# SinOncology/BreakID

Measured on AMD Instinct MI355X. Metric: M reads/s clustered+split-scanned, higher is better.
Workload: dtype int32/u8 (+f64 sd replay)

## Files before the change

### breakid_amd/capi.py

```python
from __future__ import annotations

import ctypes as C
import math
import os
import subprocess

import numpy as np

from . import abi

_HERE = os.path.dirname(os.path.abspath(__file__))
LIB_PATH = os.path.join(_HERE, "libbreakid_hip.so")
_LIB = None


class BreakIDError(RuntimeError):
    def __init__(self, code, msg):
        super().__init__("libbreakid_hip error %d: %s" % (code, msg))
        self.code = code


def build(verbose=False):
    cmd = ["make", "-C", os.path.join(_HERE, "csrc"), "-j8"]
    r = subprocess.run(cmd, capture_output=not verbose, text=True)
    if r.returncode != 0:
        raise RuntimeError("building libbreakid_hip.so failed:\n" + (r.stdout or "")[-4000:] + (r.stderr or "")[-4000:])


EXPORTS = ["bk_init", "bk_prepare_process", "bk_free", "bk_last_error", "bk_set_stream", "bk_sync", "bk_get_stream", "bk_upload_records", "bk_records", "bk_exclude_regions", "bk_isize_stats",
           "bk_discordant_pairs", "bk_mask_and_cluster", "bk_split_evidence", "bk_cluster_summary",
           "bk_split_breakpoints", "bk_normal_support", "bk_ref_support", "bk_genotype_call", "bk_clip_support", "bk_clip_reads", "bk_base_depth", "bk_clip_rescue", "bk_junctions", "bk_junction_sides", "bk_vcf_breakend_alt", "bk_evidence", "bk_run", "bk_fetch", "bk_timing", "bk_timing_enable", "bk_timing_touched", "bk_group_stats", "bk_qname_hash", "bk_qname_check",
           "bk_bam_open", "bk_bam_header", "bk_bam_decode", "bk_bam_close", "bk_bam_extract", "bk_bam_names_free", "bk_bam_decode_device", "bk_bam_decode_device_part", "bk_bam_decode_device_ctx", "bk_bam_dev_free", "bk_feed_release_caches", "bk_debug_bgzf_inflate", "bk_debug_std_sort", "bk_sort_forms", "bk_debug_ahc", "bk_debug_points", "bk_debug_cigar", "bk_debug_vote", "bk_debug_region", "bk_shard_begin", "bk_shard_get_stats", "bk_shard_set_stats",
           "bk_shard_sd_local", "bk_shard_sd_finish", "bk_shard_buffer", "bk_shard_set_buffer", "bk_shard_group_sizes",
           "bk_shard_own_groups", "bk_shard_route_candidates", "bk_shard_group_keys", "bk_shard_route_pairs", "bk_shard_group_pairs", "bk_shard_bp_cov", "bk_shard_bp_vote", "bk_shard_bp_vote_slice", "bk_shard_bp_set_voted", "bk_shard_bp_depth", "bk_shard_bp_finish"]


def lib():
    global _LIB
    if _LIB is None:
        if not os.path.exists(LIB_PATH):
            raise BreakIDError(abi.BK_ERR_NO_DEVICE, "libbreakid_hip.so is not built (run __graft_entry__.build()); "
                                                     "there is no CPU fallback")
        try:
            import torch
        except Exception:
            pass
        L = C.CDLL(LIB_PATH)
        vp, u64p, dp = C.c_void_p, C.POINTER(C.c_uint64), C.POINTER(C.c_double)
        L.bk_init.argtypes = [C.c_int, vp, C.POINTER(C.c_char_p), C.c_int, C.POINTER(vp)]
        L.bk_free.argtypes = [vp]
        L.bk_last_error.restype = C.c_char_p
        L.bk_last_error.argtypes = [vp]
        L.bk_set_stream.argtypes = [vp, vp]
        L.bk_sync.argtypes = [vp]
        L.bk_upload_records.argtypes = [vp, C.POINTER(abi.Soa), C.c_int]
        L.bk_records.argtypes = [vp, C.POINTER(abi.Soa)]
        L.bk_exclude_regions.argtypes = [vp, C.POINTER(abi.Regions), u64p]
        L.bk_isize_stats.argtypes = [vp, dp, dp]
        L.bk_discordant_pairs.argtypes = [vp, C.c_int, C.c_double, u64p, C.POINTER(C.c_uint32)]
        L.bk_mask_and_cluster.argtypes = [vp, C.c_double, C.c_int, u64p]
        L.bk_split_evidence.argtypes = [vp, u64p]
        L.bk_cluster_summary.argtypes = [vp, C.c_double, u64p]
        L.bk_split_breakpoints.argtypes = [vp, C.c_double, u64p]
        L.bk_run.argtypes = [vp, C.c_int, C.c_int, dp, u64p]
        L.bk_normal_support.argtypes = [vp, vp, C.c_double, C.POINTER(vp), u64p]
        L.bk_ref_support.argtypes = [vp, vp, C.c_int, C.c_int, C.c_double, C.POINTER(vp), u64p]
        L.bk_genotype_call.argtypes = [C.c_uint32, C.c_uint32, C.POINTER(C.c_uint8), C.POINTER(C.c_uint8), C.POINTER(C.c_float)]
        L.bk_clip_support.argtypes = [vp, vp, C.c_int, C.c_int, C.c_double, C.POINTER(vp), u64p]
        L.bk_clip_reads.argtypes = [vp, vp, C.c_uint64, C.c_int, C.c_int, C.POINTER(vp), C.POINTER(vp), C.POINTER(vp)]
        L.bk_base_depth.argtypes = [vp, vp, vp, C.c_uint64, C.POINTER(vp)]
        L.bk_clip_rescue.argtypes = [vp, vp, vp, C.c_uint32] + [C.POINTER(C.c_uint32)] * 4
        L.bk_junctions.argtypes = [vp, C.POINTER(vp), u64p]
        L.bk_junction_sides.argtypes = [vp, C.POINTER(C.c_uint8), C.POINTER(C.c_uint8), C.POINTER(C.c_uint8)]
        L.bk_vcf_breakend_alt.argtypes = [C.c_char, C.c_int, C.c_char_p, C.c_uint32, C.c_int, C.c_char_p, C.c_size_t]
        L.bk_evidence.argtypes = [vp, C.POINTER(vp), u64p, C.POINTER(C.POINTER(C.c_uint64))]
        L.bk_fetch.argtypes = [vp, C.c_int, C.POINTER(vp), u64p, C.POINTER(C.POINTER(C.c_uint64)), C.POINTER(C.c_uint32)]
        L.bk_timing.argtypes = [vp, C.POINTER(C.POINTER(C.c_char_p)), C.POINTER(C.POINTER(C.c_float)),
                                C.POINTER(C.POINTER(C.c_uint64)), C.POINTER(C.c_int)]
        L.bk_timing_enable.argtypes = [vp, C.c_int]
        L.bk_timing_touched.argtypes = [vp, C.POINTER(C.POINTER(C.c_uint64)), C.POINTER(C.c_int)]
        L.bk_debug_std_sort.argtypes = [vp, vp, vp, C.c_uint32, vp]
        L.bk_sort_forms.argtypes = [vp, u64p]
        L.bk_debug_ahc.argtypes = [vp, vp, vp, C.c_uint32, C.c_double, vp, vp, C.POINTER(C.c_uint32)]
        L.bk_debug_points.argtypes = [vp, C.c_int, vp, vp, C.c_uint32, C.c_double, vp, vp, C.POINTER(C.c_uint32)]
        L.bk_debug_cigar.argtypes = [vp, C.c_uint32, vp, vp, vp, vp, vp, vp, vp]
        L.bk_debug_vote.argtypes = [vp, vp, C.c_uint32, vp, C.c_uint32, C.c_int32, C.c_int32, vp]
        L.bk_debug_region.argtypes = [vp, C.c_int32, C.c_uint32, C.c_uint32, C.c_uint64, vp, C.c_uint32, C.POINTER(C.c_uint32), C.POINTER(C.c_uint32),
                                      C.POINTER(C.c_uint32)]
        L.bk_shard_begin.argtypes = [vp, C.c_uint64, C.c_int]
        L.bk_shard_get_stats.argtypes = [vp, C.POINTER(abi.ShardStats)]
        L.bk_shard_set_stats.argtypes = [vp, C.POINTER(abi.ShardStats)]
        L.bk_shard_sd_local.argtypes = [vp, u64p, C.POINTER(vp), u64p]
        L.bk_shard_sd_finish.argtypes = [vp, vp, C.c_uint64, C.c_uint64, dp, dp]
        L.bk_shard_buffer.argtypes = [vp, C.c_int, C.POINTER(vp), u64p, C.POINTER(C.c_uint32)]
        L.bk_shard_set_buffer.argtypes = [vp, C.c_int, vp, C.c_uint64]
        L.bk_shard_group_sizes.argtypes = [vp, C.POINTER(C.POINTER(C.c_uint64)), C.POINTER(C.c_uint32)]
        L.bk_shard_own_groups.argtypes = [vp, vp, C.c_uint32]
        L.bk_shard_route_candidates.argtypes = [vp, C.c_uint32, C.POINTER(vp), C.POINTER(C.POINTER(C.c_uint64))]
        L.bk_shard_group_keys.argtypes = [vp, C.POINTER(C.POINTER(C.c_uint32)), C.POINTER(C.c_uint32)]
        L.bk_shard_route_pairs.argtypes = [vp, vp, C.c_uint32, C.c_uint32, C.POINTER(vp), C.POINTER(C.POINTER(C.c_uint64))]
        L.bk_shard_group_pairs.argtypes = [vp, vp, C.c_uint64, vp, C.c_uint32]
        L.bk_shard_bp_cov.argtypes = [vp, C.c_double, C.POINTER(vp), u64p]
        L.bk_shard_bp_vote.argtypes = [vp, C.c_double, vp]
        L.bk_shard_bp_vote_slice.argtypes = [vp, C.c_double, vp, C.c_uint64, C.c_uint64, C.POINTER(vp), C.POINTER(vp)]
        L.bk_shard_bp_set_voted.argtypes = [vp, vp]
        L.bk_shard_bp_depth.argtypes = [vp, C.POINTER(vp), u64p]
        L.bk_shard_bp_finish.argtypes = [vp, vp]
        L.bk_qname_hash.restype = C.c_uint64
        L.bk_qname_hash.argtypes = [C.c_char_p, C.c_size_t]
        L.bk_qname_check.restype = C.c_uint32
        L.bk_qname_check.argtypes = [C.c_char_p, C.c_size_t]
        L.bk_bam_open.argtypes = [C.c_char_p, C.POINTER(vp), C.c_char_p, C.c_size_t]
        L.bk_bam_header.argtypes = [vp, C.POINTER(C.c_int), C.POINTER(C.POINTER(C.c_char_p)), C.POINTER(C.POINTER(C.c_uint32))]
        L.bk_bam_decode.argtypes = [vp, C.POINTER(abi.Soa), C.c_char_p, C.c_size_t]
        L.bk_bam_close.argtypes = [vp]
        L.bk_bam_extract.argtypes = [C.c_char_p, C.c_char_p, vp, C.c_uint64, C.POINTER(C.c_char_p), C.c_uint64, C.POINTER(vp), u64p, C.c_char_p, C.c_size_t]
        L.bk_bam_names_free.argtypes = [vp]
        L.bk_bam_names_free.restype = None
        L.bk_bam_decode_device.argtypes = [C.c_char_p, C.c_int, C.POINTER(vp), C.POINTER(abi.Soa), C.POINTER(C.c_int), C.POINTER(C.POINTER(C.c_char_p)),
                                           C.POINTER(C.POINTER(C.c_uint32)), C.c_char_p, C.c_size_t]
        L.bk_bam_decode_device_part.argtypes = [C.c_char_p, C.c_int, C.c_int, C.c_int, C.POINTER(vp), C.POINTER(abi.Soa), C.POINTER(C.c_int), C.POINTER(C.POINTER(C.c_char_p)),
                                           C.POINTER(C.POINTER(C.c_uint32)), C.c_char_p, C.c_size_t]
        L.bk_bam_dev_free.argtypes = [vp]
        L.bk_feed_release_caches.argtypes = []
        L.bk_feed_release_caches.restype = None
        L.bk_bam_decode_device_ctx.argtypes = [C.c_char_p, C.c_int, C.c_int, C.POINTER(vp), C.POINTER(vp), C.POINTER(C.c_int), C.POINTER(C.POINTER(C.c_char_p)),
                                               C.POINTER(C.POINTER(C.c_uint32)), C.c_char_p, C.c_size_t]
        L.bk_debug_bgzf_inflate.argtypes = [vp, C.c_uint64, vp, C.c_uint64, C.POINTER(C.c_uint64), C.POINTER(C.c_float), C.c_char_p, C.c_size_t]
        _LIB = L
    return _LIB


MULTI_LIB_PATH = os.path.join(_HERE, "libbreakid_rccl.so")
_MULTI = None
TRANSPORT_AUTO, TRANSPORT_RCCL, TRANSPORT_LOCAL = 0, 1, 2


def multi_lib():
    global _MULTI
    if _MULTI is None:
        lib()
        if not os.path.exists(MULTI_LIB_PATH):
            raise BreakIDError(abi.BK_ERR_NO_DEVICE, "libbreakid_rccl.so is not built (run __graft_entry__.build())")
        M = C.CDLL(MULTI_LIB_PATH)
        vp, dp = C.c_void_p, C.POINTER(C.c_double)
        M.bk_multi_run.argtypes = [C.POINTER(abi.Soa), vp, C.POINTER(C.c_char_p), C.c_int, C.c_int, C.c_int, C.c_int, C.c_int, dp, C.POINTER(C.c_uint64), C.POINTER(vp),
                                   C.c_char_p, C.c_size_t]
        M.bk_multi_stats.argtypes = [vp, dp, dp, C.POINTER(vp), C.POINTER(C.c_uint32)]
        M.bk_multi_free.argtypes = [vp]
        M.bk_multi_free.restype = None
        _MULTI = M
    return _MULTI


def multi_run(contigs, cols, n_gpus, transport=TRANSPORT_LOCAL, qual=20, fast=True):
    M = multi_lib()
    qc = cols.get("qcheck")
    cols = {k: np.ascontiguousarray(cols[k], dtype=dt) for k, dt in abi.SOA_COLS}
    if qc is not None:
        cols["qcheck"] = np.ascontiguousarray(qc, dtype=np.uint32)
    for k in ("cigar", "aux"):
        if cols[k].size == 0:
            cols[k] = np.zeros(1, cols[k].dtype)
    soa = abi.soa_from_numpy(cols)
    lens = np.asarray([l for _, l in contigs], dtype=np.uint32)
    names = (C.c_char_p * len(contigs))(*[n.encode() for n, _ in contigs])
    w, ncl, h = C.c_double(), C.c_uint64(), C.c_void_p()
    err = C.create_string_buffer(512)
    rc = M.bk_multi_run(C.byref(soa), lens.ctypes.data, names, len(contigs), int(n_gpus), int(transport), int(qual), int(fast), C.byref(w), C.byref(ncl), C.byref(h), err, 512)
    if rc != 0:
        raise BreakIDError(rc, err.value.decode())
    try:
        mean, sd = C.c_double(), C.c_double()
        rc = M.bk_multi_stats(h, C.byref(mean), C.byref(sd), None, None)
        if rc != 0:
            raise BreakIDError(rc, "bk_multi_stats")
        L = lib()
        clusters, _ = abi.fetch_array(L, h, lambda hh, st, d, c, g, ng: L.bk_fetch(hh, st, d, c, g, ng), abi.STAGE_CLUSTERS)
        return {"w": w.value, "n_clustered": ncl.value, "mean": mean.value, "sd": sd.value, "clusters": clusters}
    finally:
        M.bk_multi_free(h)


def w_from(mean, sd):
    times = 2
    return times * math.sqrt(times) * (mean + 3 * sd)


def genotype_call(alt, ref):
    gt, gq, vaf = C.c_uint8(), C.c_uint8(), C.c_float()
    rc = lib().bk_genotype_call(int(alt), int(ref), C.byref(gt), C.byref(gq), C.byref(vaf))
    if rc != 0:
        raise BreakIDError(rc, "bk_genotype_call")
    return gt.value, gq.value, np.float32(vaf.value)


def junction_sides(row):
    a = np.zeros(1, abi.JUNCTION)
    a[0] = row
    r1, r2, src = C.c_uint8(), C.c_uint8(), C.c_uint8()
    rc = lib().bk_junction_sides(a.ctypes.data, C.byref(r1), C.byref(r2), C.byref(src))
    if rc != 0:
        raise BreakIDError(rc, "bk_junction_sides")
    return r1.value, r2.value, src.value


def clip_rescue(cluster, junction, clip, min_support=3):
    c, j, s = np.zeros(1, abi.CLUSTER), np.zeros(1, abi.JUNCTION), np.zeros(1, abi.CLIP_SUPPORT)
    c[0], j[0], s[0] = cluster, junction, clip
    out = [C.c_uint32() for _ in range(4)]
    rc = lib().bk_clip_rescue(c.ctypes.data, j.ctypes.data, s.ctypes.data, int(min_support), *[C.byref(o) for o in out])
    if rc < 0:
        raise BreakIDError(rc, "bk_clip_rescue")
    return tuple(o.value for o in out) if rc == 1 else None


def vcf_breakend_alt(ref_base, own_right, mate_chr, mate_pos, mate_right, cap=None):
    chrom = mate_chr.encode()
    if cap is None:
        cap = len(chrom) + 32
    buf = C.create_string_buffer(max(int(cap), 1))
    rc = lib().bk_vcf_breakend_alt(ref_base.encode(), int(bool(own_right)), chrom, int(mate_pos), int(bool(mate_right)), buf, int(cap))
    if rc != 0:
        raise BreakIDError(rc, "bk_vcf_breakend_alt")
    return buf.value.decode()


class Context:

    def __init__(self, contigs, device=0):
        self.L = lib()
        self.contigs = list(contigs)
        lens = np.asarray([l for _, l in contigs], dtype=np.uint32)
        names = (C.c_char_p * len(contigs))(*[n.encode() for n, _ in contigs])
        h = C.c_void_p()
        rc = self.L.bk_init(device, lens.ctypes.data, names, len(contigs), C.byref(h))
        if rc != 0:
            raise BreakIDError(rc, (self.L.bk_last_error(None) or b"").decode())
        self.h = h
        self._keep = None

    def close(self):
        if self.h:
            self.L.bk_free(self.h)
            self.h = None

    def __del__(self):
        try:
            self.close()
        except Exception:
            pass

    def _check(self, rc):
        if rc != 0:
            raise BreakIDError(rc, (self.L.bk_last_error(self.h) or b"").decode())

    def set_stream(self, hip_stream_handle):
        self._check(self.L.bk_set_stream(self.h, C.c_void_p(hip_stream_handle)))

    def sync(self):
        self._check(self.L.bk_sync(self.h))

    def upload(self, cols):
        qc = cols.get("qcheck")
        cols = {k: np.ascontiguousarray(cols[k], dtype=dt) for k, dt in abi.SOA_COLS}
        if qc is not None:
            cols["qcheck"] = np.ascontiguousarray(qc, dtype=np.uint32)
        for k in ("cigar", "aux"):
            if cols[k].size == 0:
                cols[k] = np.zeros(1, cols[k].dtype)
        soa = abi.soa_from_numpy(cols)
        self._keep = (cols, soa)
        self._check(self.L.bk_upload_records(self.h, C.byref(soa), abi.BK_MEM_HOST))

    def attach_device_table(self, table):
        self._keep = table
        self._check(self.L.bk_upload_records(self.h, C.byref(table.soa), abi.BK_MEM_DEVICE))

    def upload_soa(self, handle):
# ... 384 lines not shown
```

### breakid_amd/csrc/lanes.hip

```cpp
#include <algorithm>
#include <atomic>
#include <chrono>
#include <cmath>
#include <cstdio>
#include <numeric>
#include <thread>
#include <dirent.h>

#include "lanes.h"

static int g_hw_queues_at_init = 0;
void stage_set_hw_queues(int n) { g_hw_queues_at_init = n; }

static bool sort_service_on()
{
  static const bool on = !(getenv("BREAKID_SORT_SERVICE") && atoi(getenv("BREAKID_SORT_SERVICE")) == 0);
  return on;
}
constexpr int LANE_STREAMS_MAX = 4;
constexpr int SVC_STAGE_QUEUES = LANE_STREAMS_MAX + 3;
static bool lane_service(int fast) { return sort_service_on() && fast && g_hw_queues_at_init >= SVC_STAGE_QUEUES; }
static int stage_queues() { return std::max(1, g_hw_queues_at_init - 1); }
static int lane_streams_each(int K)
{
  static const int want = getenv("BREAKID_LANE_STREAMS") ? atoi(getenv("BREAKID_LANE_STREAMS")) : 0;
  if (want == 1 || want == 2) return want;
  return stage_queues() >= 2 * K ? 2 : 1;
}
static int lanes_wanted(bool svc)
{
  const char *env = getenv("BREAKID_GROUP_LANES");
  static const int want_svc = env ? atoi(env) : 12;
  if (svc) return want_svc < 1 ? 1 : (want_svc > 26 ? 26 : want_svc);
  static const int want = env ? atoi(env) : std::max(1, std::min(4, stage_queues() / lane_streams_each(std::min(4, stage_queues()))));
  return want < 1 ? 1 : (want > 26 ? 26 : want);
}
static bool lanes_apply(const StageInput &in, int fast)
{
  static const uint64_t min_pairs = getenv("BREAKID_LANES_MIN_PAIRS") ? strtoull(getenv("BREAKID_LANES_MIN_PAIRS"), nullptr, 10) : (1ull << 20);
  uint32_t large = 0;
  const uint64_t big = std::max<uint64_t>(2, min_pairs >> 6);
  for (uint32_t g = 0; g < in.jr.n_groups && g + 1 < in.gstart_host.size(); ++g) large += in.gstart_host[g + 1] - in.gstart_host[g] >= big ? 1u : 0u;
  const bool yes = lanes_wanted(lane_service(fast)) >= 2 && fast && in.jr.n_groups >= 4 && in.jr.n_pairs >= min_pairs && large >= 2;
  if (yes)
  {
    static bool told = false;
    const int K = lanes_wanted(lane_service(fast));
    if (!told && !lane_service(fast) && K * lane_streams_each(K) > stage_queues() && bk_debug("lanes"))
    {
      told = true;
      fprintf(stderr, "[breakid] GPU_MAX_HW_QUEUES=%d: the lanes of chromosome-pair groups (bk_mask_and_cluster) and their heap kernels will share hardware queues "
                        "(BREAKID_GROUP_LANES=1: one pass)\n", g_hw_queues_at_init);
    }
  }
  return yes;
}

__global__ void k_svc_probe() {}
static int kfd_compute_queues(int device)
{
  char bus[64] = {0};
  if (hipDeviceGetPCIBusId(bus, (int) sizeof bus, device) != hipSuccess) return -1;
  unsigned dom = 0, b = 0, d = 0, f = 0;
  if (sscanf(bus, "%x:%x:%x.%x", &dom, &b, &d, &f) != 4) return -1;
  const unsigned long want_loc = (b << 8) | (d << 3) | f;
  auto read_file = [](const std::string &path, std::string &out) {
    FILE *fp = fopen(path.c_str(), "r");
    if (!fp) return false;
    char buf[4096];
    const size_t n = fread(buf, 1, sizeof buf - 1, fp);
    fclose(fp);
    buf[n] = 0;
    out = buf;
    return true;
  };
  auto list_dir = [](const std::string &path, std::vector<std::string> &names) {
    DIR *dp = opendir(path.c_str());
    if (!dp) return false;
    while (dirent *e = readdir(dp))
      if (e->d_name[0] != '.') names.push_back(e->d_name);
    closedir(dp);
    return true;
  };
  unsigned long gpu_id = 0;
  {
    std::vector<std::string> nodes;
    if (!list_dir("/sys/class/kfd/kfd/topology/nodes", nodes)) return -1;
    for (const std::string &n : nodes)
// ... 120 lines not shown
    return ok && took < 0.003;
  }
  void set(SortService *s)
  {
    for (auto &l : cs.lanes)
    {
      l->cb.se.svc = s;
      l->cb.se.svc_slot = 0xFFFFFFFFu;
    }
  }
  void finish()
  {
    if (!on) return;
    on = false;
    set(nullptr);
    hipError_t e = hipStreamSynchronize(st);
    for (auto &l : cs.lanes)
      if (l->st && e == hipSuccess) e = hipStreamSynchronize(l->st);
    cs.svc.stop();
    device_turn.unlock();
    if (e != hipSuccess) throw bk_error(BK_ERR_HIP, std::string("sort service: ") + hipGetErrorString(e));
  }
  ~SvcStage()
  {
    try
    {
      finish();
    }
    catch (const bk_error &)
    {
    }
  }
};

static void snapshot_list(const PairList &L, DevBuf &idx, DevBuf *gof, DevBuf &goff, hipStream_t st)
{
  uint32_t *ii = idx.as<uint32_t>(L.n + 1), *ig = gof ? gof->as<uint32_t>(L.n + 1) : nullptr;
  uint64_t *io = goff.as<uint64_t>((uint64_t) L.ng + 1);
  if (L.n) HIP_CHECK(hipMemcpyAsync(ii, L.idx.get<uint32_t>(), L.n * 4, hipMemcpyDeviceToDevice, st));
  if (L.n && ig) HIP_CHECK(hipMemcpyAsync(ig, L.gof.get<uint32_t>(), L.n * 4, hipMemcpyDeviceToDevice, st));
  if (L.ng) HIP_CHECK(hipMemcpyAsync(io, L.goff.get<uint64_t>(), ((uint64_t) L.ng + 1) * 8, hipMemcpyDeviceToDevice, st));
}
static void cluster_list(const bk_pair *pairs, PairList &L, double w, int fast, DevBuf &cl, ClusterBufs &cb, AhcBufs &ab, hipStream_t st)
{
  if (fast)
    fast_cluster_all(pairs, L, w, cl, cb, st);
  else
    ahc_cluster_all(pairs, L, w, cl, ab, cb, st);
}

using LanePlan = std::vector<int>;
static LanePlan plan_owned(const StageInput &in)
{
  const uint32_t ng = in.jr.n_groups;
  const bool owned_only = !in.own_groups.empty();
  if (owned_only && in.own_groups.size() != ng) throw bk_error(BK_ERR_ARG, "bk_shard_own_groups: group count changed");
  LanePlan p(ng, 0);
  for (uint32_t g = 0; owned_only && g < ng; ++g)
    if (!in.own_groups[g]) p[g] = -1;
  return p;
}
static LanePlan plan_blind(const StageInput &in, int K)
{
  const uint32_t ng = in.jr.n_groups;
  std::vector<uint32_t> order(ng);
  std::iota(order.begin(), order.end(), 0u);
  auto size_of = [&](uint32_t g) { return in.gstart_host[g + 1] - in.gstart_host[g]; };
  std::stable_sort(order.begin(), order.end(), [&](uint32_t a, uint32_t b) { return size_of(a) > size_of(b); });
  constexpr double wexp = 2.0;
  LanePlan p = plan_owned(in);
  std::vector<double> load(K, 0.0);
  for (uint32_t i = 0; i < ng; ++i)
  {
    const uint32_t g = order[i];
    if (p[g] < 0) continue;
    int l = 0;
    for (int k = 1; k < K; ++k)
      if (load[k] < load[l]) l = k;
    load[l] += std::pow((double) size_of(g), wexp);
    p[g] = l;
  }
  return p;
}
static LanePlan plan_observed(const std::vector<uint64_t> &sizes, const std::vector<uint32_t> &hx, const std::vector<uint32_t> &hy, int K)
{
  const uint32_t ng = (uint32_t) sizes.size();
  constexpr double per_pair = 0.001;
  auto heap_cost = [](uint32_t m) { return (double) m + (m > 40947u ? 1.0 * (double) (m - 40947u) : 0.0); };
  std::vector<uint32_t> order(ng);
  std::iota(order.begin(), order.end(), 0u);
  auto chain = [&](uint32_t g) { return heap_cost(hx[g]) + heap_cost(hy[g]); };
  std::stable_sort(order.begin(), order.end(), [&](uint32_t a, uint32_t b) {
    const double ca = chain(a), cb = chain(b);
    return ca != cb ? ca > cb : sizes[a] > sizes[b];
  });
  LanePlan p(ng, 0);
  std::vector<double> mx(K, 0.0), my(K, 0.0), pairs(K, 0.0);
  auto cost = [&](int l) { return mx[l] + my[l] + per_pair * pairs[l]; };
  for (uint32_t g : order)
  {
    int best = 0;
    double best_cost = 0;
    for (int l = 0; l < K; ++l)
    {
      const double c = std::max(mx[l], heap_cost(hx[g])) + std::max(my[l], heap_cost(hy[g])) + per_pair * (pairs[l] + (double) sizes[g]);
      if (l == 0 || c < best_cost || (c == best_cost && cost(l) < cost(best)))
      {
        best = l;
        best_cost = c;
      }
    }
    mx[best] = std::max(mx[best], heap_cost(hx[g]));
    my[best] = std::max(my[best], heap_cost(hy[g]));
    pairs[best] += (double) sizes[g];
    p[g] = best;
  }
  if (bk_debug("lanes"))
    for (int l = 0; l < K; ++l)
    {
      fprintf(stderr, "[lanes] lane %d: max heap x %.0f y %.0f, %.0f pairs, cost %.0f; heavy groups:", l, mx[l], my[l], pairs[l], cost(l));
      for (uint32_t g = 0; g < ng; ++g)
        if (p[g] == l && (hx[g] || hy[g])) fprintf(stderr, " %u(%u,%u)", g, hx[g], hy[g]);
      fprintf(stderr, "\n");
    }
  return p;
}
static uint32_t *upload_drop(const LanePlan &p, int K, DevBuf &buf, hipStream_t st)
{
  const size_t row = p.size() + 1;
  std::vector<uint32_t> drop((size_t) K * row, 0u);
  for (int l = 0; l < K; ++l)
    for (size_t g = 0; g + 1 < row; ++g) drop[(size_t) l * row + g] = p[g] == l ? 0u : 1u;
  uint32_t *d = buf.as<uint32_t>(drop.size() + 1);
  HIP_CHECK(hipMemcpyAsync(d, drop.data(), drop.size() * 4, hipMemcpyHostToDevice, st));
  HIP_CHECK(hipStreamSynchronize(st));
  return d;
}

static void group_lanes(ClusterStage &cs, const StageInput &in, double w, int fast)
{
  const uint32_t ng = in.jr.n_groups;
  static const bool dbg = bk_debug("lanes");
  auto make_lanes = [&](int K, int S) {
    while ((int) cs.lanes.size() < K)
    {
      cs.lanes.emplace_back(new ClusterStage::Lane());
      cs.lanes.back()->cb.max_group_bound = cs.cb().max_group_bound;
    }
    for (int k = 1; k < S; ++k)
      if (!cs.lanes[k]->st) HIP_CHECK(hipStreamCreateWithFlags(&cs.lanes[k]->st, hipStreamNonBlocking));
  };
  bool use_svc = sort_service_on() && fast;
  if (use_svc && !lane_service(fast))
  {
    use_svc = false;
    tell_no_service();
    if (bk_debug("lanes")) fprintf(stderr, "[lanes] %d hardware queues, the sort service needs %d: not started\n", g_hw_queues_at_init, SVC_STAGE_QUEUES);
  }
  int K = lanes_wanted(use_svc);
  int S = use_svc ? std::max(1, std::min(LANE_STREAMS_MAX, K)) : K;
  make_lanes(K, S);
  std::vector<hipStream_t> stage_streams{in.st};
  for (int k = 1; k < S; ++k) stage_streams.push_back(cs.lanes[k]->st);
  SvcStage svc_stage(cs, in.device, in.st, use_svc, in.jr.n_pairs + 2ull * ng + 4096, cs.cb().max_group_bound, stage_streams);
  if (use_svc && !svc_stage.on)
  {
    use_svc = false;
    K = lanes_wanted(false);
    S = K;
    make_lanes(K, S);
  }
  struct ForkReset
  {
    ClusterBufs &cb;
    ~ForkReset() { cb.se.fork_heaps = true; }
  } fork_reset{cs.cb()};
  {
    const bool fork = use_svc || lane_streams_each(K) == 2;
    for (int k = 0; k < K; ++k) cs.lanes[k]->cb.se.fork_heaps = fork;
    if (!use_svc && bk_debug("lanes")) fprintf(stderr, "[lanes] launch path: %d lanes, %d stream%s each, %d hardware queues\n", K, fork ? 2 : 1, fork ? "s" : "", g_hw_queues_at_init);
    if (!use_svc && sort_tasks_on() && bk_debug("lanes")) fprintf(stderr, "[lanes] sorts as task dispatches on the lane streams\n");
  }
  auto lane = [&](int l) -> ClusterStage::Lane & { return *cs.lanes[l]; };
  auto lane_st = [&](int l) { const int k = l % S; return k == 0 ? in.st : cs.lanes[k]->st; };
  uint32_t *drop_base = nullptr;
  auto lane_drop = [&](int l) { return drop_base + (size_t) l * ((size_t) ng + 1); };
  std::vector<std::vector<uint8_t>> keep(K, std::vector<uint8_t>(ng, 0));
  auto upload_plan = [&](const LanePlan &p) {
    for (int l = 0; l < K; ++l)
      for (uint32_t g = 0; g < ng; ++g) keep[l][g] = p[g] == l ? 1 : 0;
    drop_base = upload_drop(p, K, cs.d_drop, in.st);
  };
  auto in_lanes = [&](auto body) {
    std::vector<std::string> err(K);
    std::vector<int> code(K, BK_OK);
    const auto t_start = std::chrono::steady_clock::now();
    auto guarded_body = [&](int l) {
      try
      {
        body(l);
        HIP_CHECK(hipStreamSynchronize(lane_st(l)));
        if (dbg)
          fprintf(stderr, "[lanes] lane %d done after %.2f ms\n", l, std::chrono::duration<double, std::milli>(std::chrono::steady_clock::now() - t_start).count());
      }
      catch (const bk_error &e)
      {
        code[l] = e.code;
        err[l] = e.msg;
// ... 131 lines not shown
```

### include/breakid_hip.h

```cpp
#ifndef BREAKID_HIP_H
#define BREAKID_HIP_H

#include <stdint.h>
#include <stddef.h>

#ifdef __cplusplus
extern "C" {
#endif

#define BK_OK 0
#define BK_ERR_ARG (-1)
#define BK_ERR_HIP (-2)
#define BK_ERR_NO_DEVICE (-3)
#define BK_ERR_UNSORTED (-4)
#define BK_ERR_CIGAR (-5)
#define BK_ERR_IO (-6)
#define BK_ERR_LIMIT (-7)
#define BK_ERR_COLLISION (-8)

#define BK_MEM_HOST 0
#define BK_MEM_DEVICE 1

typedef struct bk_ctx bk_ctx;

// ... 115 lines not shown
int bk_clip_support(bk_ctx *calls, bk_ctx *records, int mapq_min, int min_clip, double w, const struct bk_clip_support **out, uint64_t *count);
int bk_base_depth(bk_ctx *records, const int32_t *tid, const uint32_t *pos, uint64_t n, const uint32_t **out);
int bk_clip_rescue(const bk_cluster *c, const struct bk_junction *j, const struct bk_clip_support *s, uint32_t min_support, uint32_t *pos1, uint32_t *pos2, uint32_t *n1,
                   uint32_t *n2);

struct bk_clip_site { int32_t tid; uint32_t pos; uint32_t tol; uint32_t dir; };
struct bk_clip_read {
  uint64_t rec;
  uint64_t qhash;
  uint32_t qcheck;
  uint32_t site;
  int32_t tid; uint32_t p;
  uint32_t clip_len;
  uint16_t flag;
  uint8_t mapq;
  uint8_t dir;
};
int bk_clip_reads(bk_ctx *records, const struct bk_clip_site *sites, uint64_t n_sites, int mapq_min, int min_clip, const uint32_t **counts,
                  const struct bk_clip_read **rows, const uint64_t **site_off);

#define BK_EV_PAIR 1
#define BK_EV_SPLIT 2
struct bk_evidence {
  uint64_t rec;
  uint64_t qhash;
  uint32_t qcheck;
  uint32_t call;
  int32_t tid1; uint32_t pos1;
  int32_t tid2; uint32_t pos2;
  uint16_t flag1, flag2;
  uint8_t mapq1, mapq2;
  uint8_t kind;
  uint8_t sides;
};
int bk_evidence(bk_ctx *ctx, const struct bk_evidence **out, uint64_t *count, const uint64_t **call_off);

int bk_fetch(bk_ctx *ctx, int stage, const void **data, uint64_t *count, const uint64_t **group_off, uint32_t *n_groups);

typedef struct bk_group_stat {
  int32_t p1_tid, p2_tid;
  uint64_t n_scan, n_isolated_removed, n_clustered;
  uint32_t cluster_id_end;
  uint32_t ordinal;
} bk_group_stat;
int bk_group_stats(bk_ctx *ctx, const bk_group_stat **out, uint32_t *n_groups);

int bk_timing(bk_ctx *ctx, const char *const **names, const float **ms, const uint64_t **bytes, int *n);
int bk_timing_enable(bk_ctx *ctx, int on);
int bk_timing_touched(bk_ctx *ctx, const uint64_t **touched, int *n);

typedef struct bk_shard_stats {
  uint64_t isize_sum, isize_n;
  double sumsq;
  uint32_t vmax, max_span;
  uint64_t n_cand, n_split;
} bk_shard_stats;
#define BK_BUF_CANDIDATES 0
#define BK_BUF_TUPLES 1
#define BK_BUF_CLUSTERS 2
int bk_shard_begin(bk_ctx *ctx, uint64_t rec_base, int mapq_min);
int bk_shard_get_stats(bk_ctx *ctx, bk_shard_stats *out);
int bk_shard_set_stats(bk_ctx *ctx, const bk_shard_stats *total);
int bk_shard_sd_local(bk_ctx *ctx, uint64_t *l_total, void **ex_dev, uint64_t *n_ex);
int bk_shard_sd_finish(bk_ctx *ctx, const void *all_ex_dev, uint64_t n_all, uint64_t l_grand, double *mean, double *sd);
int bk_shard_buffer(bk_ctx *ctx, int which, void **dev, uint64_t *count, uint32_t *elem_bytes);
int bk_shard_set_buffer(bk_ctx *ctx, int which, const void *dev, uint64_t count);
int bk_shard_group_sizes(bk_ctx *ctx, const uint64_t **starts, uint32_t *n_groups);
int bk_shard_own_groups(bk_ctx *ctx, const uint8_t *own, uint32_t n_groups);
int bk_shard_route_candidates(bk_ctx *ctx, uint32_t world, void **dev, const uint64_t **counts);
int bk_shard_group_keys(bk_ctx *ctx, const uint32_t **keys, uint32_t *n_groups);
int bk_shard_route_pairs(bk_ctx *ctx, const uint32_t *dest_of_group, uint32_t n_groups, uint32_t world, void **dev, const uint64_t **counts);
int bk_shard_group_pairs(bk_ctx *ctx, const void *pairs_dev, uint64_t n, const uint32_t *all_keys, uint32_t n_all_keys);
int bk_shard_bp_cov(bk_ctx *ctx, double w, void **cov_dev, uint64_t *n);
int bk_shard_bp_vote(bk_ctx *ctx, double w, const void *cov_total_dev);
int bk_shard_bp_vote_slice(bk_ctx *ctx, double w, const void *cov_total_dev, uint64_t lo, uint64_t hi, void **clusters_dev, void **voted_dev);
int bk_shard_bp_set_voted(bk_ctx *ctx, const void *voted_all_dev);
int bk_shard_bp_depth(bk_ctx *ctx, void **depth_dev, uint64_t *n);
int bk_shard_bp_finish(bk_ctx *ctx, const void *depth_total_dev);

int bk_debug_std_sort(bk_ctx *ctx, const uint32_t *key, const uint64_t *group_off, uint32_t n_groups, uint32_t *perm_out);

int bk_sort_forms(bk_ctx *ctx, uint64_t out[3]);

int bk_debug_ahc(bk_ctx *ctx, const uint32_t *x, const uint32_t *y, uint32_t n, double w, uint32_t *idx_out, int32_t *cluster_out, uint32_t *n_out);

int bk_debug_points(bk_ctx *ctx, int mode, const uint32_t *x, const uint32_t *y, uint32_t n, double w, uint32_t *idx_out, int32_t *cluster_out, uint32_t *n_out);
int bk_debug_cigar(bk_ctx *ctx, uint32_t n, const uint8_t *kind, const uint32_t *c1_off, const uint8_t *c1, const uint32_t *c2_off, const uint8_t *c2, const int32_t *e,
                   int32_t *out6);
int bk_debug_vote(bk_ctx *ctx, const bk_split *side1, uint32_t n1, const bk_split *side2, uint32_t n2, int32_t p1_tid, int32_t p2_tid, int32_t *out3);
int bk_debug_region(bk_ctx *ctx, int32_t tid, uint32_t start, uint32_t end, uint64_t depth_pos, bk_split *out, uint32_t cap, uint32_t *n_out, uint32_t *cov_out,
                    uint32_t *depth_out);

typedef struct bk_bam bk_bam;
uint64_t bk_qname_hash(const char *name, size_t len);
uint32_t bk_qname_check(const char *name, size_t len);
int bk_bam_open(const char *path, bk_bam **out, char *err, size_t errlen);
int bk_bam_header(const bk_bam *b, int *n_targets, const char *const **names, const uint32_t **lens);
int bk_bam_decode(bk_bam *b, bk_soa *out, char *err, size_t errlen);
void bk_bam_close(bk_bam *b);
typedef struct bk_read_key { uint64_t qhash; uint32_t qcheck; uint32_t tag; } bk_read_key;
int bk_bam_extract(const char *in_bam, const char *out_bam, const bk_read_key *keys, uint64_t n_keys, const char *const *tags, uint64_t n_tags, char **names_out,
                   uint64_t *n_written, char *err, size_t errlen);
void bk_bam_names_free(char *names);

typedef struct bk_bam_dev bk_bam_dev;
int bk_bam_decode_device(const char *path, int device, bk_bam_dev **out, bk_soa *cols, int *n_targets, const char *const **names, const uint32_t **lens,
                         char *err, size_t errlen);
int bk_bam_decode_device_part(const char *path, int device, int part, int parts, bk_bam_dev **out, bk_soa *cols, int *n_targets, const char *const **names,
                              const uint32_t **lens, char *err, size_t errlen);
void bk_bam_dev_free(bk_bam_dev *h);
void bk_feed_release_caches(void);
int bk_bam_decode_device_ctx(const char *path, int device, int mapq_min, bk_bam_dev **bam_out, bk_ctx **ctx_out, int *n_targets, const char *const **names,
                             const uint32_t **lens, char *err, size_t errlen);
int bk_records(bk_ctx *ctx, bk_soa *cols);
int bk_debug_bgzf_inflate(const void *file, uint64_t n, void *out, uint64_t out_cap, uint64_t *out_len, float *kernel_ms, char *err, size_t errlen);

#ifdef __cplusplus
}
#endif
#endif
```

Baseline: 11760.

## Assign cluster groups to lanes with a fitted cost model and local search

Replaces the greedy assignment of groups to parallel lanes with a model-based search. It starts from the greedy plan, then repeatedly moves or swaps heavy heap groups and re-deals bulk groups to minimise the modelled worst lane time. The aim is to cut the critical lane in the clustering stage. The trade-off is extra host-side planning work and reliance on hand-fitted timing constants that may not match other inputs. A greedy fallback environment switch and a debug entry point are added.

```diff
diff --git a/breakid_amd/capi.py b/breakid_amd/capi.py
--- a/breakid_amd/capi.py
+++ b/breakid_amd/capi.py
@@ -30,7 +30,7 @@
 EXPORTS = ["bk_init", "bk_prepare_process", "bk_free", "bk_last_error", "bk_set_stream", "bk_sync", "bk_get_stream", "bk_upload_records", "bk_records", "bk_exclude_regions", "bk_isize_stats",
            "bk_discordant_pairs", "bk_mask_and_cluster", "bk_split_evidence", "bk_cluster_summary",
            "bk_split_breakpoints", "bk_normal_support", "bk_ref_support", "bk_genotype_call", "bk_clip_support", "bk_clip_reads", "bk_base_depth", "bk_clip_rescue", "bk_junctions", "bk_junction_sides", "bk_vcf_breakend_alt", "bk_evidence", "bk_run", "bk_fetch", "bk_timing", "bk_timing_enable", "bk_timing_touched", "bk_group_stats", "bk_qname_hash", "bk_qname_check",
-           "bk_bam_open", "bk_bam_header", "bk_bam_decode", "bk_bam_close", "bk_bam_extract", "bk_bam_names_free", "bk_bam_decode_device", "bk_bam_decode_device_part", "bk_bam_decode_device_ctx", "bk_bam_dev_free", "bk_feed_release_caches", "bk_debug_bgzf_inflate", "bk_debug_std_sort", "bk_sort_forms", "bk_debug_ahc", "bk_debug_points", "bk_debug_cigar", "bk_debug_vote", "bk_debug_region", "bk_shard_begin", "bk_shard_get_stats", "bk_shard_set_stats",
+           "bk_bam_open", "bk_bam_header", "bk_bam_decode", "bk_bam_close", "bk_bam_extract", "bk_bam_names_free", "bk_bam_decode_device", "bk_bam_decode_device_part", "bk_bam_decode_device_ctx", "bk_bam_dev_free", "bk_feed_release_caches", "bk_debug_bgzf_inflate", "bk_debug_std_sort", "bk_sort_forms", "bk_debug_ahc", "bk_debug_points", "bk_debug_cigar", "bk_debug_vote", "bk_debug_region", "bk_debug_plan_lanes", "bk_shard_begin", "bk_shard_get_stats", "bk_shard_set_stats",
            "bk_shard_sd_local", "bk_shard_sd_finish", "bk_shard_buffer", "bk_shard_set_buffer", "bk_shard_group_sizes",
            "bk_shard_own_groups", "bk_shard_route_candidates", "bk_shard_group_keys", "bk_shard_route_pairs", "bk_shard_group_pairs", "bk_shard_bp_cov", "bk_shard_bp_vote", "bk_shard_bp_vote_slice", "bk_shard_bp_set_voted", "bk_shard_bp_depth", "bk_shard_bp_finish"]
 
@@ -87,6 +87,7 @@
         L.bk_debug_vote.argtypes = [vp, vp, C.c_uint32, vp, C.c_uint32, C.c_int32, C.c_int32, vp]
         L.bk_debug_region.argtypes = [vp, C.c_int32, C.c_uint32, C.c_uint32, C.c_uint64, vp, C.c_uint32, C.POINTER(C.c_uint32), C.POINTER(C.c_uint32),
                                       C.POINTER(C.c_uint32)]
+        L.bk_debug_plan_lanes.argtypes = [vp, vp, vp, C.c_uint32, C.c_int, C.c_int, vp, vp]
         L.bk_shard_begin.argtypes = [vp, C.c_uint64, C.c_int]
         L.bk_shard_get_stats.argtypes = [vp, C.POINTER(abi.ShardStats)]
         L.bk_shard_set_stats.argtypes = [vp, C.POINTER(abi.ShardStats)]
@@ -195,6 +196,20 @@
     return gt.value, gq.value, np.float32(vaf.value)
 
 
+def debug_plan_lanes(sizes, hx, hy, K, greedy=False):
+    sizes = np.ascontiguousarray(sizes, dtype=np.uint64)
+    hx = np.ascontiguousarray(hx, dtype=np.uint32)
+    hy = np.ascontiguousarray(hy, dtype=np.uint32)
+    if not (len(sizes) == len(hx) == len(hy)):
+        raise ValueError("debug_plan_lanes: sizes, hx and hy differ in length")
+    lane = np.empty(len(sizes), np.int32)
+    ms = np.empty(max(int(K), 1), np.float64)
+    rc = lib().bk_debug_plan_lanes(sizes.ctypes.data, hx.ctypes.data, hy.ctypes.data, len(sizes), int(K), int(bool(greedy)), lane.ctypes.data, ms.ctypes.data)
+    if rc != 0:
+        raise BreakIDError(rc, "bk_debug_plan_lanes")
+    return lane, ms
+
+
 def junction_sides(row):
     a = np.zeros(1, abi.JUNCTION)
     a[0] = row
diff --git a/breakid_amd/csrc/lanes.hip b/breakid_amd/csrc/lanes.hip
--- a/breakid_amd/csrc/lanes.hip
+++ b/breakid_amd/csrc/lanes.hip
@@ -4,6 +4,7 @@
 #include <cmath>
 #include <cstdio>
 #include <numeric>
+#include <string>
 #include <thread>
 #include <dirent.h>
 
@@ -290,11 +291,11 @@
   }
   return p;
 }
-static LanePlan plan_observed(const std::vector<uint64_t> &sizes, const std::vector<uint32_t> &hx, const std::vector<uint32_t> &hy, int K)
+static double heap_cost(uint32_t m) { return (double) m + (m > 40947u ? 1.0 * (double) (m - 40947u) : 0.0); }
+static LanePlan deal_greedy(const std::vector<uint64_t> &sizes, const std::vector<uint32_t> &hx, const std::vector<uint32_t> &hy, int K)
 {
   const uint32_t ng = (uint32_t) sizes.size();
   constexpr double per_pair = 0.001;
-  auto heap_cost = [](uint32_t m) { return (double) m + (m > 40947u ? 1.0 * (double) (m - 40947u) : 0.0); };
   std::vector<uint32_t> order(ng);
   std::iota(order.begin(), order.end(), 0u);
   auto chain = [&](uint32_t g) { return heap_cost(hx[g]) + heap_cost(hy[g]); };
@@ -323,15 +324,213 @@
     pairs[best] += (double) sizes[g];
     p[g] = best;
   }
+  return p;
+}
+
+namespace lane_model
+{
+constexpr double P0 = 1.40, P1 = 0.44e-6;
+constexpr double S0 = 1.15;
+constexpr double POP_Y = 0.160e-3, POP_X = 0.178e-3;
+constexpr double G0 = 1.43, G1 = 0.29e-6;
+}
+static double lane_time(double pairs, uint32_t hx_max, uint32_t hy_max)
+{
+  using namespace lane_model;
+  const double part = P0 + P1 * pairs;
+  return G0 + G1 * pairs + std::max(part, S0 + POP_Y * heap_cost(hy_max)) + std::max(part, S0 + POP_X * heap_cost(hx_max));
+}
+struct LaneLoads
+{
+  struct Score
+  {
+    double worst = 0, sum = 0;
+    bool better_than(double worst_b, double sum_b) const
+    {
+      constexpr double eps = 1e-9;
+      return worst < worst_b - eps || (worst <= worst_b + eps && sum < sum_b - eps);
+    }
+  };
+  std::vector<double> pairs, ms;
+  std::vector<uint32_t> hx, hy;
+  double worst = 0, sum = 0;
+  explicit LaneLoads(int K) : pairs(K, 0.0), ms(K, 0.0), hx(K, 0u), hy(K, 0u) {}
+  void time()
+  {
+    worst = sum = 0;
+    for (size_t l = 0; l < ms.size(); ++l)
+    {
+      ms[l] = lane_time(pairs[l], hx[l], hy[l]);
+      worst = std::max(worst, ms[l]);
+      sum += ms[l];
+    }
+  }
+  bool better_than(double worst_b, double sum_b) const { return Score{worst, sum}.better_than(worst_b, sum_b); }
+};
+static LaneLoads lane_loads(const LanePlan &p, const std::vector<uint64_t> &sizes, const std::vector<uint32_t> &hx, const std::vector<uint32_t> &hy, int K)
+{
+  LaneLoads L(K);
+  for (size_t g = 0; g < p.size(); ++g)
+  {
+    const int l = p[g];
+    L.pairs[l] += (double) sizes[g];
+    L.hx[l] = std::max(L.hx[l], hx[g]);
+    L.hy[l] = std::max(L.hy[l], hy[g]);
+  }
+  L.time();
+  return L;
+}
+static LanePlan deal_modelled(const std::vector<uint64_t> &sizes, const std::vector<uint32_t> &hx, const std::vector<uint32_t> &hy, int K)
+{
+  constexpr uint32_t DEAL_HEAVY_MAX = 32;
+  constexpr int DEAL_STEPS_MAX = 64, DEAL_ROUNDS_MAX = 8;
+  const uint32_t ng = (uint32_t) sizes.size();
+  LanePlan p = deal_greedy(sizes, hx, hy, K);
+  if (K < 2 || ng < 2) return p;
+  std::vector<uint32_t> heavy, bulk;
+  for (uint32_t g = 0; g < ng; ++g) (hx[g] || hy[g] ? heavy : bulk).push_back(g);
+  auto chain = [&](uint32_t g) { return heap_cost(hx[g]) + heap_cost(hy[g]); };
+  std::stable_sort(heavy.begin(), heavy.end(), [&](uint32_t a, uint32_t b) { return chain(a) > chain(b); });
+  std::stable_sort(bulk.begin(), bulk.end(), [&](uint32_t a, uint32_t b) { return sizes[a] > sizes[b]; });
+  const uint32_t nh = std::min<uint32_t>((uint32_t) heavy.size(), DEAL_HEAVY_MAX);
+  struct Top2
+  {
+    uint32_t a = 0, b = 0;
+    void add(uint32_t v)
+    {
+      if (v > a)
+        b = a, a = v;
+      else if (v > b)
+        b = v;
+    }
+    uint32_t without(uint32_t v) const { return v == a ? b : a; }
+  };
+  std::vector<Top2> tx(K), ty(K);
+  LaneLoads cur(K);
+  auto heaps_step = [&] {
+    bool gained = false;
+    for (int step = 0; step < DEAL_STEPS_MAX; ++step)
+    {
+      cur = lane_loads(p, sizes, hx, hy, K);
+      tx.assign(K, Top2());
+      ty.assign(K, Top2());
+      for (uint32_t g = 0; g < ng; ++g)
+        if (hx[g] || hy[g]) tx[p[g]].add(hx[g]), ty[p[g]].add(hy[g]);
+      double best_worst = cur.worst, best_sum = cur.sum;
+      uint32_t ba = nh, bb = nh;
+      int bB = 0;
+      auto consider = [&](uint32_t a, uint32_t b, int B) {
+        const uint32_t ga = heavy[a], gb = b != nh ? heavy[b] : 0;
+        const int A = p[ga];
+        const double sa = (double) sizes[ga], sb = b != nh ? (double) sizes[gb] : 0.0;
+        const uint32_t bx = b != nh ? hx[gb] : 0u, by = b != nh ? hy[gb] : 0u;
+        const double ms_a = lane_time(cur.pairs[A] - sa + sb, std::max(tx[A].without(hx[ga]), bx), std::max(ty[A].without(hy[ga]), by));
+        const double ms_b = lane_time(cur.pairs[B] + sa - sb, std::max(b != nh ? tx[B].without(bx) : tx[B].a, hx[ga]), std::max(b != nh ? ty[B].without(by) : ty[B].a, hy[ga]));
+        LaneLoads::Score c{std::max(ms_a, ms_b), ms_a + ms_b};
+        for (int l = 0; l < K; ++l)
+          if (l != A && l != B) c.worst = std::max(c.worst, cur.ms[l]), c.sum += cur.ms[l];
+        if (!c.better_than(best_worst, best_sum)) return;
+        best_worst = c.worst, best_sum = c.sum;
+        ba = a, bb = b, bB = B;
+      };
+      for (uint32_t a = 0; a < nh; ++a)
+        for (int l = 0; l < K; ++l)
+          if (l != p[heavy[a]]) consider(a, nh, l);
+      for (uint32_t a = 0; a < nh; ++a)
+        for (uint32_t b = a + 1; b < nh; ++b)
+          if (p[heavy[a]] != p[heavy[b]]) consider(a, b, p[heavy[b]]);
+      if (ba == nh) break;
+      if (bb != nh) p[heavy[bb]] = p[heavy[ba]];
+      p[heavy[ba]] = bB;
+      gained = true;
+    }
+    return gained;
+  };
+  auto bulk_step = [&] {
+    if (bulk.empty()) return false;
+    const LaneLoads before = lane_loads(p, sizes, hx, hy, K);
+    LaneLoads L = before;
+    for (uint32_t g : bulk) L.pairs[p[g]] -= (double) sizes[g];
+    L.time();
+    std::vector<int> to(bulk.size());
+    for (size_t i = 0; i < bulk.size(); ++i)
+    {
+      const double s = (double) sizes[bulk[i]];
+      int w1 = 0;
+      for (int l = 1; l < K; ++l)
+        if (L.ms[l] > L.ms[w1]) w1 = l;
+      double second = 0;
+      for (int l = 0; l < K; ++l)
+        if (l != w1) second = std::max(second, L.ms[l]);
+      int best = -1;
+      LaneLoads::Score best_score;
+      double best_ms = 0;
+      for (int l = 0; l < K; ++l)
+      {
+        const double ms = lane_time(L.pairs[l] + s, L.hx[l], L.hy[l]);
+        const LaneLoads::Score c{std::max(ms, l == w1 ? second : L.ms[w1]), L.sum - L.ms[l] + ms};
+        if (best < 0 || c.better_than(best_score.worst, best_score.sum)) best = l, best_score = c, best_ms = ms;
+      }
+      to[i] = best;
+      L.pairs[best] += s;
+      L.sum += best_ms - L.ms[best];
+      L.ms[best] = best_ms;
+    }
+    L.time();
+    if (!L.better_than(before.worst, before.sum)) return false;
+    for (size_t i = 0; i < bulk.size(); ++i) p[bulk[i]] = to[i];
+    return true;
+  };
+  for (int round = 0; round < DEAL_ROUNDS_MAX; ++round)
+  {
+    const bool b = bulk_step();
+    const bool a = nh ? heaps_step() : false;
+    if (!a && !b) break;
+  }
+  return p;
+}
+static bool deal_greedy_only()
+{
+  static const bool greedy = getenv("BREAKID_LANE_DEAL") && std::string(getenv("BREAKID_LANE_DEAL")) == "greedy";
+  return greedy;
+}
+static LanePlan plan_observed(const std::vector<uint64_t> &sizes, const std::vector<uint32_t> &hx, const std::vector<uint32_t> &hy, int K)
+{
+  const uint32_t ng = (uint32_t) sizes.size();
+  const bool greedy = deal_greedy_only();
+  const LanePlan p = greedy ? deal_greedy(sizes, hx, hy, K) : deal_modelled(sizes, hx, hy, K);
   if (bk_debug("lanes"))
+  {
+    const LaneLoads L = lane_loads(p, sizes, hx, hy, K);
     for (int l = 0; l < K; ++l)
     {
-      fprintf(stderr, "[lanes] lane %d: max heap x %.0f y %.0f, %.0f pairs, cost %.0f; heavy groups:", l, mx[l], my[l], pairs[l], cost(l));
+      const double mx = heap_cost(L.hx[l]), my = heap_cost(L.hy[l]);
+      fprintf(stderr, "[lanes] lane %d: max heap x %.0f y %.0f, %.0f pairs, cost %.0f; heavy groups:", l, mx, my, L.pairs[l], mx + my + 0.001 * L.pairs[l]);
       for (uint32_t g = 0; g < ng; ++g)
         if (p[g] == l && (hx[g] || hy[g])) fprintf(stderr, " %u(%u,%u)", g, hx[g], hy[g]);
       fprintf(stderr, "\n");
     }
+    for (int l = 0; l < K; ++l) fprintf(stderr, "[lanes] lane %d: modelled %.2f ms for part 2 (%s deal)\n", l, L.ms[l], greedy ? "greedy" : "modelled");
+  }
   return p;
+}
+extern "C" int bk_debug_plan_lanes(const uint64_t *sizes, const uint32_t *hx, const uint32_t *hy, uint32_t ng, int K, int greedy, int32_t *lane_out, double *lane_ms_out)
+{
+  if (K < 1 || K > 26 || !lane_ms_out || (ng && (!sizes || !hx || !hy || !lane_out))) return BK_ERR_ARG;
+  try
+  {
+    const std::vector<uint64_t> s(sizes, sizes + ng);
+    const std::vector<uint32_t> x(hx, hx + ng), y(hy, hy + ng);
+    const LanePlan p = greedy ? deal_greedy(s, x, y, K) : deal_modelled(s, x, y, K);
+    const LaneLoads L = lane_loads(p, s, x, y, K);
+    for (uint32_t g = 0; g < ng; ++g) lane_out[g] = p[g];
+    for (int l = 0; l < K; ++l) lane_ms_out[l] = L.ms[l];
+    return BK_OK;
+  }
+  catch (const std::exception &)
+  {
+    return BK_ERR_ARG;
+  }
 }
 static uint32_t *upload_drop(const LanePlan &p, int K, DevBuf &buf, hipStream_t st)
 {
diff --git a/include/breakid_hip.h b/include/breakid_hip.h
--- a/include/breakid_hip.h
+++ b/include/breakid_hip.h
@@ -221,6 +221,8 @@
 
 int bk_sort_forms(bk_ctx *ctx, uint64_t out[3]);
 
+int bk_debug_plan_lanes(const uint64_t *sizes, const uint32_t *hx, const uint32_t *hy, uint32_t ng, int K, int greedy, int32_t *lane_out, double *lane_ms_out);
+
 int bk_debug_ahc(bk_ctx *ctx, const uint32_t *x, const uint32_t *y, uint32_t n, double w, uint32_t *idx_out, int32_t *cluster_out, uint32_t *n_out);
 
 int bk_debug_points(bk_ctx *ctx, int mode, const uint32_t *x, const uint32_t *y, uint32_t n, double w, uint32_t *idx_out, int32_t *cluster_out, uint32_t *n_out);
```

New measurement: 12170, median of 6. +3.5%, better.
